# rishabhjain16/audio-visual-llm

Hardware: AMD Instinct MI355X
Metric: AV-clip train-step samples/sec (clip_whisper -> Llama-2-7B LoRA), whole job (higher is better)
Workload: dtype bf16

## Files before the change

### audio-visual-llm_amd/csrc/elementwise.hip

```cpp
#include "common.h"
#include "avllm_internal.h"

namespace {

template <typename T>
__global__ void rope_kernel(T* __restrict__ x, long ld, long rows, int T_, int heads, int hd, int pos0, float theta, int inverse) {
    const int half = hd >> 1;
    const long total = rows * heads * (half >> 2);
    for (long idx = blockIdx.x * (long)blockDim.x + threadIdx.x; idx < total; idx += (long)gridDim.x * blockDim.x) {
        const int qd = (int)(idx % (half >> 2));
        const int h = (int)((idx / (half >> 2)) % heads);
        const long row = idx / ((long)(half >> 2) * heads);
        const int pos = pos0 + (int)(row % T_);
        T* p = x + row * ld + (long)h * hd + qd * 4;
        float a[4], b[4], oa[4], ob[4];
        load_f<4>(p, a);
        load_f<4>(p + half, b);
#pragma unroll
        for (int j = 0; j < 4; ++j) {
            const int i = qd * 4 + j;
            const float inv = 1.0f / powf(theta, (float)(2 * i) / (float)hd);
            const float ang = (float)pos * inv;
            float c = cosf(ang), s = sinf(ang);
            if (inverse) s = -s;
// ... 206 lines not shown
        cols[(idx / w) * Kpad + K + idx % w] = from_f<T>(0.f);
}
template <typename T>
__global__ void cls_rows_kernel(const T* __restrict__ ce, const T* __restrict__ pos, T* __restrict__ x, int N, int tokens, int d) {
    const long total = (long)N * (d >> 2);
    for (long idx = blockIdx.x * (long)blockDim.x + threadIdx.x; idx < total; idx += (long)gridDim.x * blockDim.x) {
        const long n = idx / (d >> 2);
        const int c = (int)(idx % (d >> 2)) * 4;
        float a[4], b[4];
        load_f<4>(ce + c, a);
        load_f<4>(pos + c, b);
#pragma unroll
        for (int j = 0; j < 4; ++j) a[j] += b[j];
        store_f<4>(x + n * tokens * d + c, a);
    }
}

template <typename T>
__device__ __forceinline__ void virt_row(const T* a, int Ta, const T* v, int Tv, const T* pe, int P, int L, int b, int j, int c,
                                         int D, float fs, float (&o)[4]) {
    o[0] = o[1] = o[2] = o[3] = 0.f;
    if (j < P) { load_f<4>(pe + ((long)b * P + j) * D + c, o); return; }
    const int t = j - P;
    if (a && v) {
        float t4[4];
        if (t < Ta) { load_f<4>(a + ((long)b * Ta + t) * D + c, t4);
#pragma unroll
            for (int k = 0; k < 4; ++k) o[k] = fs * t4[k]; }
        if (t < Tv) { load_f<4>(v + ((long)b * Tv + t) * D + c, t4);
#pragma unroll
            for (int k = 0; k < 4; ++k) o[k] += (1.0f - fs) * t4[k]; }
    } else if (a) { if (t < Ta) load_f<4>(a + ((long)b * Ta + t) * D + c, o); }
    else { if (t < Tv) load_f<4>(v + ((long)b * Tv + t) * D + c, o); }
}

template <typename T>
__global__ void fuse_pool_kernel(const T* __restrict__ a, int Ta, const T* __restrict__ v, int Tv, const T* __restrict__ pe,
                                 int P, T* __restrict__ out, int L, int S_out, int D, float fs) {
    const int b = blockIdx.y, i = blockIdx.x;
    const int Lt = P + L;
    for (int c = threadIdx.x * 4; c < D; c += blockDim.x * 4) {
        float acc[4] = {0.f, 0.f, 0.f, 0.f}, r[4];
        if (Lt == S_out) {
            virt_row(a, Ta, v, Tv, pe, P, L, b, i, c, D, fs, acc);
        } else if (Lt > S_out) {
            const int s = (int)(((long)i * Lt) / S_out);
            const int e = (int)((((long)(i + 1)) * Lt + S_out - 1) / S_out);
            for (int j = s; j < e; ++j) {
                virt_row(a, Ta, v, Tv, pe, P, L, b, j, c, D, fs, r);
#pragma unroll
                for (int k = 0; k < 4; ++k) acc[k] += r[k];
            }
            const float cnt = (float)(e - s);
#pragma unroll
            for (int k = 0; k < 4; ++k) acc[k] = acc[k] / cnt;
        } else {
            const float scale = S_out > 1 ? (float)(Lt - 1) / (float)(S_out - 1) : 0.f;
            const float src = scale * i;
            const int lo = (int)src;
            const int hi = lo + 1 < Lt ? lo + 1 : Lt - 1;
            const float w1 = src - (float)lo, w0 = 1.0f - w1;
            float r2[4];
            virt_row(a, Ta, v, Tv, pe, P, L, b, lo, c, D, fs, r);
            virt_row(a, Ta, v, Tv, pe, P, L, b, hi, c, D, fs, r2);
#pragma unroll
            for (int k = 0; k < 4; ++k) acc[k] = w0 * r[k] + w1 * r2[k];
        }
        store_f<4>(out + ((long)b * S_out + i) * D + c, acc);
    }
}

template <typename T, int VEC>
__global__ void fuse_pool_bwd_kernel(const T* __restrict__ dx, T* __restrict__ da, int Ta, T* __restrict__ dv, int Tv, int P, int L,
                                     int S_out, int D, float fs) {
    const int b = blockIdx.y, t = blockIdx.x;
    const int Lt = P + L, j = P + t;
    const bool both = Ta > 0 && Tv > 0;
    const float scale = (Lt < S_out && S_out > 1) ? (float)(Lt - 1) / (float)(S_out - 1) : 0.f;
    int i0 = 0, i1 = -1;
    if (t < L) {
        if (Lt == S_out) { i0 = i1 = j; }
        else if (Lt > S_out) {
            i0 = (int)(((long)j * S_out) / Lt);
            i1 = (int)((((long)(j + 1)) * S_out - 1) / Lt);
        } else if (scale > 0.f) {
            i0 = (int)floorf((float)(j - 1) / scale) - 1;
            i1 = (int)ceilf((float)(j + 1) / scale) + 1;
        } else { i0 = 0; i1 = S_out - 1; }
        i0 = i0 < 0 ? 0 : i0;
        i1 = i1 > S_out - 1 ? S_out - 1 : i1;
    }
    for (int c = (int)threadIdx.x * VEC; c < D; c += (int)blockDim.x * VEC) {
        float g[VEC], r[VEC];
#pragma unroll
        for (int k = 0; k < VEC; ++k) g[k] = 0.f;
        for (int i = i0; i <= i1; ++i) {
            const T* src = dx + ((long)b * S_out + i) * D + c;
            if (Lt == S_out) {
                load_f<VEC>(src, g);
            } else if (Lt > S_out) {
                const int s = (int)(((long)i * Lt) / S_out);
                const int e = (int)((((long)(i + 1)) * Lt + S_out - 1) / S_out);
                if (j < s || j >= e) continue;
                const float cnt = (float)(e - s);
                load_f<VEC>(src, r);
#pragma unroll
                for (int k = 0; k < VEC; ++k) g[k] += r[k] / cnt;
            } else {
                const float sp = scale * i;
                const int lo = (int)sp;
                const int hi = lo + 1 < Lt ? lo + 1 : Lt - 1;
                if (lo != j && hi != j) continue;
                const float w1 = sp - (float)lo, w0 = 1.0f - w1;
                const float wgt = (lo == j ? w0 : 0.f) + (hi == j ? w1 : 0.f);
                load_f<VEC>(src, r);
#pragma unroll
                for (int k = 0; k < VEC; ++k) g[k] += wgt * r[k];
            }
        }
        if (da && t < Ta) {
#pragma unroll
            for (int k = 0; k < VEC; ++k) r[k] = both ? fs * g[k] : g[k];
            store_f<VEC>(da + ((long)b * Ta + t) * D + c, r);
        }
        if (dv && t < Tv) {
#pragma unroll
            for (int k = 0; k < VEC; ++k) r[k] = both ? (1.0f - fs) * g[k] : g[k];
            store_f<VEC>(dv + ((long)b * Tv + t) * D + c, r);
        }
    }
}

template <typename T>
__global__ void lora_pack_kernel(const float* __restrict__ A, const float* __restrict__ Bm, int r, int din, int dout,
                                 T* __restrict__ A_pad, T* __restrict__ AT_pad, long ld_at, T* __restrict__ B_pad, T* __restrict__ BT_pad) {
    const long nA = (long)AVLLM_LORA_PAD * din, nB = (long)AVLLM_LORA_PAD * dout;
    for (long idx = blockIdx.x * (long)blockDim.x + threadIdx.x; idx < nA + nB; idx += (long)gridDim.x * blockDim.x) {
        if (idx < nA) {
            const int j = (int)(idx / din), k = (int)(idx % din);
            const float val = j < r ? A[(long)j * din + k] : 0.f;
            A_pad[(long)j * din + k] = from_f<T>(val);
            AT_pad[(long)k * ld_at + j] = from_f<T>(val);
        } else {
            const long i2 = idx - nA;
            const int j = (int)(i2 / dout), n = (int)(i2 % dout);
            const float val = j < r ? Bm[(long)n * r + j] : 0.f;
            BT_pad[(long)j * dout + n] = from_f<T>(val);
            B_pad[(long)n * AVLLM_LORA_PAD + j] = from_f<T>(val);
        }
    }
}

template <typename T>
__global__ void lora_pack_batch_kernel(const avllm_lora_pack_item* __restrict__ items, int r, int din) {
    const avllm_lora_pack_item it = items[blockIdx.x];
    const int dout = (int)it.dout;
    const long nA = (long)r * din, nB = (long)r * dout;
    T* A_pad = (T*)it.A_pad; T* AT_pad = (T*)it.AT_pad; T* B_pad = (T*)it.B_pad; T* BT_pad = (T*)it.BT_pad;
    for (long idx = blockIdx.y * (long)blockDim.x + threadIdx.x; idx < nA + nB; idx += (long)gridDim.y * blockDim.x) {
        if (idx < nA) {
            const int j = (int)(idx / din), k = (int)(idx % din);
            const float val = it.A[(long)j * din + k];
            A_pad[(long)j * din + k] = from_f<T>(val);
            AT_pad[(long)k * it.ld_at + j] = from_f<T>(val);
        } else {
            const long i2 = idx - nA;
            const int j = (int)(i2 / dout), n = (int)(i2 % dout);
            const float val = it.B[(long)n * r + j];
            BT_pad[(long)j * dout + n] = from_f<T>(val);
            B_pad[(long)n * AVLLM_LORA_PAD + j] = from_f<T>(val);
        }
    }
}

template <typename T>
__global__ void kv_append_kernel(const T* __restrict__ k, const T* __restrict__ v, long ld, T* __restrict__ kc, T* __restrict__ vc,
                                 int B, int Tn, int pos0, int Tmax, int d) {
    const long total = (long)B * Tn * (d >> 2);
    for (long idx = blockIdx.x * (long)blockDim.x + threadIdx.x; idx < total; idx += (long)gridDim.x * blockDim.x) {
        const int c = (int)(idx % (d >> 2)) * 4;
        const long row = idx / (d >> 2);
        const int b = (int)(row / Tn), t = (int)(row % Tn);
        float x[4];
        load_f<4>(k + row * ld + c, x);
        store_f<4>(kc + ((long)b * Tmax + pos0 + t) * d + c, x);
        load_f<4>(v + row * ld + c, x);
        store_f<4>(vc + ((long)b * Tmax + pos0 + t) * d + c, x);
    }
}

inline int grid_for(long total, int block = 256) {
    long g = (total + block - 1) / block;
    return (int)(g < 1 ? 1 : (g > 8192 ? 8192 : g));
}

}

int av_rope(void* x, long ld, long rows, int T, int heads, int hd, int pos0, float theta, int inverse, int dtype, hipStream_t st) {
    AV_CHECK_ARG(x && rows > 0 && T > 0, "rope: null/empty");
    AV_CHECK_ARG(hd % 8 == 0 && ld % 4 == 0, "rope: head_dim %d must be a multiple of 8", hd);
    const long total = rows * heads * (hd / 8);
    if (dtype == AV_F32) hipLaunchKernelGGL((rope_kernel<float>), dim3(grid_for(total)), dim3(256), 0, st, (float*)x, ld, rows, T, heads, hd, pos0, theta, inverse);
    else hipLaunchKernelGGL((rope_kernel<bf16>), dim3(grid_for(total)), dim3(256), 0, st, (bf16*)x, ld, rows, T, heads, hd, pos0, theta, inverse);
    AV_LAUNCH_CHECK();
    return AV_OK;
}

int av_rope_table(float* tab, int T, int hd, int pos0, float theta, hipStream_t st, const int* pos_dev, AvRopeScale sc) {
    AV_CHECK_ARG(tab && T > 0 && hd % 8 == 0, "rope_table: bad args");
    hipLaunchKernelGGL(rope_table_kernel, dim3(av_cdiv((long)T * (hd / 2), 256)), dim3(256), 0, st, tab, T, hd, pos0, theta, pos_dev, sc);
    AV_LAUNCH_CHECK();
    return AV_OK;
}

int av_rope_tab(void* x, long ld, long rows, int T, int heads, int hd, const float* tab, int inverse, int dtype, hipStream_t st) {
    AV_CHECK_ARG(x && tab && rows > 0 && T > 0 && hd % 8 == 0 && ld % 4 == 0, "rope(tab): bad args");
    const long total = rows * heads * (hd / 8);
    if (dtype == AV_F32) hipLaunchKernelGGL((rope_tab_kernel<float>), dim3(grid_for(total)), dim3(256), 0, st, (float*)x, ld, rows, T, heads, hd, tab, inverse);
    else hipLaunchKernelGGL((rope_tab_kernel<bf16>), dim3(grid_for(total)), dim3(256), 0, st, (bf16*)x, ld, rows, T, heads, hd, tab, inverse);
    AV_LAUNCH_CHECK();
    return AV_OK;
}

int av_swiglu_fwd(const void* gu, void* h, long M, int F, int dtype, hipStream_t st) {
    AV_CHECK_ARG(gu && h && M > 0 && F % 4 == 0, "swiglu_fwd: bad args");
    if (dtype == AV_F32) hipLaunchKernelGGL((swiglu_fwd_kernel<float>), dim3(grid_for(M * (F / 4))), dim3(256), 0, st, (const float*)gu, (float*)h, M, F);
    else hipLaunchKernelGGL((swiglu_fwd_kernel<bf16>), dim3(grid_for(M * (F / 4))), dim3(256), 0, st, (const bf16*)gu, (bf16*)h, M, F);
    AV_LAUNCH_CHECK();
    return AV_OK;
}

int av_swiglu_bwd(const void* dh, const void* gu, void* dgu, long M, int F, int dtype, hipStream_t st) {
    AV_CHECK_ARG(dh && gu && dgu && M > 0 && F % 4 == 0, "swiglu_bwd: bad args");
    if (dtype == AV_F32) hipLaunchKernelGGL((swiglu_bwd_kernel<float, false>), dim3(grid_for(M * (F / 4))), dim3(256), 0, st, (const float*)dh, (const float*)gu, (float*)dgu, (float*)nullptr, M, F);
    else hipLaunchKernelGGL((swiglu_bwd_kernel<bf16, false>), dim3(grid_for(M * (F / 4))), dim3(256), 0, st, (const bf16*)dh, (const bf16*)gu, (bf16*)dgu, (bf16*)nullptr, M, F);
    AV_LAUNCH_CHECK();
    return AV_OK;
}

int av_swiglu_bwd_h(const void* dh, const void* gu, void* dgu, void* h, long M, int F, int dtype, hipStream_t st) {
    AV_CHECK_ARG(dh && gu && dgu && h && M > 0 && F > 0 && F % 4 == 0, "swiglu_bwd_h: bad args");
    AV_CHECK_ARG(dtype == AV_F32 || dtype == AV_BF16, "swiglu_bwd_h: dtype %d", dtype);
    if (dtype == AV_F32) hipLaunchKernelGGL((swiglu_bwd_kernel<float, true>), dim3(grid_for(M * (F / 4))), dim3(256), 0, st, (const float*)dh, (const float*)gu, (float*)dgu, (float*)h, M, F);
    else hipLaunchKernelGGL((swiglu_bwd_kernel<bf16, true>), dim3(grid_for(M * (F / 4))), dim3(256), 0, st, (const bf16*)dh, (const bf16*)gu, (bf16*)dgu, (bf16*)h, M, F);
    AV_LAUNCH_CHECK();
    return AV_OK;
}

int av_act_residual(const void* x, const void* r, void* y, long n, int act, int dtype, hipStream_t st) {
    AV_CHECK_ARG(x && y && n > 0 && n % 4 == 0, "act_residual: bad args (n=%ld must be a multiple of 4)", n);
    if (dtype == AV_F32) hipLaunchKernelGGL((act_residual_kernel<float>), dim3(grid_for(n / 4)), dim3(256), 0, st, (const float*)x, (const float*)r, (float*)y, n / 4, act);
    else hipLaunchKernelGGL((act_residual_kernel<bf16>), dim3(grid_for(n / 4)), dim3(256), 0, st, (const bf16*)x, (const bf16*)r, (bf16*)y, n / 4, act);
    AV_LAUNCH_CHECK();
    return AV_OK;
}

int av_dropout(const void* x, void* y, long rows, int d, uint32_t seed, float p, int dtype, hipStream_t st, const uint32_t* seed_dev) {
    AV_CHECK_ARG(x && y && rows > 0 && d % 4 == 0 && p >= 0.f && p < 1.f, "dropout: bad args");
    const long total = rows * (d / 4);
    if (dtype == AV_F32) hipLaunchKernelGGL((dropout_kernel<float>), dim3(grid_for(total)), dim3(256), 0, st, (const float*)x, (float*)y, rows, d, seed, p, seed_dev);
    else hipLaunchKernelGGL((dropout_kernel<bf16>), dim3(grid_for(total)), dim3(256), 0, st, (const bf16*)x, (bf16*)y, rows, d, seed, p, seed_dev);
    AV_LAUNCH_CHECK();
    return AV_OK;
}

int av_embedding(const void* table, const int64_t* ids, void* out, long n, int d, int dtype, hipStream_t st) {
    AV_CHECK_ARG(table && ids && out && n > 0 && d % 4 == 0, "embedding: bad args");
    if (dtype == AV_F32) hipLaunchKernelGGL((embedding_kernel<float>), dim3(grid_for(n * (d / 4))), dim3(256), 0, st, (const float*)table, ids, (float*)out, n, d);
    else hipLaunchKernelGGL((embedding_kernel<bf16>), dim3(grid_for(n * (d / 4))), dim3(256), 0, st, (const bf16*)table, ids, (bf16*)out, n, d);
    AV_LAUNCH_CHECK();
    return AV_OK;
}

int av_cast(const void* src, int sdt, void* dst, int ddt, long n, hipStream_t st) {
    AV_CHECK_ARG(src && dst && n > 0, "cast: bad args");
    const dim3 g(grid_for(n / 4 + 1)), b(256);
    if (sdt == AV_F32 && ddt == AV_BF16) hipLaunchKernelGGL((cast_kernel<float, bf16>), g, b, 0, st, (const float*)src, (bf16*)dst, n);
    else if (sdt == AV_BF16 && ddt == AV_F32) hipLaunchKernelGGL((cast_kernel<bf16, float>), g, b, 0, st, (const bf16*)src, (float*)dst, n);
    else if (sdt == AV_F32 && ddt == AV_F32) hipLaunchKernelGGL((cast_kernel<float, float>), g, b, 0, st, (const float*)src, (float*)dst, n);
    else if (sdt == AV_BF16 && ddt == AV_BF16) hipLaunchKernelGGL((cast_kernel<bf16, bf16>), g, b, 0, st, (const bf16*)src, (bf16*)dst, n);
    else return av_set_error(AV_ERR_ARG, "cast: dtype %d->%d", sdt, ddt);
    AV_LAUNCH_CHECK();
    return AV_OK;
}

int av_whisper_im2col1(const float* mel, void* cols, int B, int n_mels, int T, int Kpad, int dtype, hipStream_t st) {
    AV_CHECK_ARG(mel && cols && B > 0 && T > 0, "im2col1: bad args");
    AV_CHECK_ARG(Kpad % 4 == 0 && Kpad >= n_mels * 3, "im2col1: Kpad=%d too small", Kpad);
    const size_t sh = (size_t)n_mels * 68 * sizeof(float);
    if (dtype == AV_F32) hipLaunchKernelGGL((im2col1_kernel<float>), dim3(av_cdiv(T, 64), B), dim3(256), sh, st, mel, (float*)cols, n_mels, T, Kpad);
    else hipLaunchKernelGGL((im2col1_kernel<bf16>), dim3(av_cdiv(T, 64), B), dim3(256), sh, st, mel, (bf16*)cols, n_mels, T, Kpad);
    AV_LAUNCH_CHECK();
    return AV_OK;
}

int av_whisper_im2col2(const void* h, void* cols, int B, int T, int d, int dtype, hipStream_t st) {
    AV_CHECK_ARG(h && cols && B > 0 && T % 2 == 0 && d % 8 == 0, "im2col2: bad args");
    const long total = (long)B * (T / 2) * 3 * (d / 8);
    if (dtype == AV_F32) hipLaunchKernelGGL((im2col2_kernel<float>), dim3(grid_for(total)), dim3(256), 0, st, (const float*)h, (float*)cols, B, T, d);
    else hipLaunchKernelGGL((im2col2_kernel<bf16>), dim3(grid_for(total)), dim3(256), 0, st, (const bf16*)h, (bf16*)cols, B, T, d);
    AV_LAUNCH_CHECK();
    return AV_OK;
}

int av_clip_patchify(const void* frames, void* cols, int N, int S, int p, int Kpad, int dtype, hipStream_t st, int in_dtype) {
    AV_CHECK_ARG(frames && cols && N > 0, "patchify: bad args");
    AV_CHECK_ARG(p > 0 && S % p == 0, "patchify: image %d is not a whole number of %d-pixel patches", S, p);
    const int K = 3 * p * p;
    AV_CHECK_ARG(Kpad >= K && Kpad % 4 == 0, "patchify: Kpad=%d < %d", Kpad, K);
    const int V = p % 4 == 0 ? 4 : p % 2 == 0 ? 2 : 1;
    const long total = (long)N * 3 * S * (S / V);
    const long rows = (long)N * (S / p) * (S / p);
#define AV_PATCHIFY(T, VV) do { if (in_dtype == AV_BF16) hipLaunchKernelGGL((patchify_kernel<T, VV, bf16>), dim3(grid_for(total)), dim3(256), 0, st, (const bf16*)frames, (T*)cols, N, S, p, Kpad); \
                                else hipLaunchKernelGGL((patchify_kernel<T, VV, float>), dim3(grid_for(total)), dim3(256), 0, st, (const float*)frames, (T*)cols, N, S, p, Kpad); } while (0)
    if (dtype == AV_F32) {
        if (V == 4) AV_PATCHIFY(float, 4); else if (V == 2) AV_PATCHIFY(float, 2); else AV_PATCHIFY(float, 1);
        if (Kpad > K) hipLaunchKernelGGL((patchify_pad_kernel<float>), dim3(grid_for(rows * (Kpad - K))), dim3(256), 0, st, (float*)cols, rows, K, Kpad);
    } else {
        if (V == 4) AV_PATCHIFY(bf16, 4); else if (V == 2) AV_PATCHIFY(bf16, 2); else AV_PATCHIFY(bf16, 1);
        if (Kpad > K) hipLaunchKernelGGL((patchify_pad_kernel<bf16>), dim3(grid_for(rows * (Kpad - K))), dim3(256), 0, st, (bf16*)cols, rows, K, Kpad);
    }
#undef AV_PATCHIFY
    AV_LAUNCH_CHECK();
// ... 67 lines not shown
```

### audio-visual-llm_amd/csrc/lora_batch.hip

```cpp
#include "common.h"
#include "avllm_internal.h"

namespace {

constexpr int RK_WAVES = 8;

struct Rank3Args {
    const bf16* A[3]; long lda[3]; int K[3];
    const bf16* B[3]; long ldb[3];
    bf16* C[3]; long ldc[3];
    uint32_t seed[3];
    int nj, M;
    float alpha, p;
    const uint32_t* seed_dev;
};

__device__ __forceinline__ bf16x8 rk_drop(bf16x8 x, uint32_t seed, unsigned long long idx0, uint32_t thr, float sc) {
    float v[8];
#pragma unroll
    for (int j = 0; j < 8; ++j) v[j] = (float)x[j];
    av_mask8(v, seed, idx0, thr, sc);
    bf16x8 r;
#pragma unroll
    for (int j = 0; j < 8; ++j) r[j] = (bf16)v[j];
    return r;
}

template <bool SHARED, bool DROP, int NJ>
__global__ __launch_bounds__(RK_WAVES * 64) void lora_rank3_kernel(Rank3Args a) {
    __shared__ float part[NJ][RK_WAVES][16][17];
    const int lane = threadIdx.x & 63, w = threadIdx.x >> 6;
    const int fr = lane & 15, fq = lane >> 4;
    const int m0 = blockIdx.x * 16;
    const int j0 = SHARED ? 0 : blockIdx.y;
    int ar = m0 + fr; ar = ar < a.M ? ar : a.M - 1;
    const int K = a.K[j0], kw = K / RK_WAVES;
    const bf16* ap = a.A[j0] + (long)ar * a.lda[j0] + (long)w * kw + fq * 8;
    const bf16* bp[NJ];
    uint32_t seed[NJ];
    f32x4 acc[NJ];
#pragma unroll
    for (int j = 0; j < NJ; ++j) {
        bp[j] = a.B[j0 + j] + (long)fr * a.ldb[j0 + j] + (long)w * kw + fq * 8;
        seed[j] = DROP ? av_seed(a.seed_dev, a.seed[j0 + j]) : 0u;
        acc[j] = (f32x4){0.f, 0.f, 0.f, 0.f};
    }
    const uint32_t thr = av_drop_thr(a.p);
    const float dsc = av_drop_scale(a.p);
    const unsigned long long idx_base = (unsigned long long)ar * K + (unsigned long long)w * kw + fq * 8;
    constexpr int UNR = 4;
    int k = 0;
    for (; k + 32 * UNR <= kw; k += 32 * UNR) {
        bf16x8 xa[UNR], wb[UNR][NJ];
#pragma unroll
        for (int u = 0; u < UNR; ++u) {
            xa[u] = *(const bf16x8*)(ap + k + 32 * u);
#pragma unroll
            for (int j = 0; j < NJ; ++j) wb[u][j] = *(const bf16x8*)(bp[j] + k + 32 * u);
        }
#pragma unroll
        for (int u = 0; u < UNR; ++u)
#pragma unroll
            for (int j = 0; j < NJ; ++j) {
                const bf16x8 x = DROP ? rk_drop(xa[u], seed[j], idx_base + k + 32 * u, thr, dsc) : xa[u];
                acc[j] = __builtin_amdgcn_mfma_f32_16x16x32_bf16(wb[u][j], x, acc[j], 0, 0, 0);
            }
    }
    for (; k < kw; k += 32) {
        const bf16x8 xa = *(const bf16x8*)(ap + k);
#pragma unroll
        for (int j = 0; j < NJ; ++j) {
            const bf16x8 wb = *(const bf16x8*)(bp[j] + k);
            const bf16x8 x = DROP ? rk_drop(xa, seed[j], idx_base + k, thr, dsc) : xa;
            acc[j] = __builtin_amdgcn_mfma_f32_16x16x32_bf16(wb, x, acc[j], 0, 0, 0);
        }
    }
#pragma unroll
    for (int j = 0; j < NJ; ++j)
#pragma unroll
        for (int i = 0; i < 4; ++i) part[j][w][fr][fq * 4 + i] = acc[j][i];
    __syncthreads();
    for (int e = threadIdx.x; e < NJ * 16 * 64; e += RK_WAVES * 64) {
        const int j = e / (16 * 64), r = (e >> 6) & 15, c = e & 63;
        if (m0 + r >= a.M) continue;
        float s = 0.f;
        if (c < 16) {
#pragma unroll
            for (int x = 0; x < RK_WAVES; ++x) s += part[j][x][r][c];
            s *= a.alpha;
        }
        a.C[j0 + j][(long)(m0 + r) * a.ldc[j0 + j] + c] = (bf16)s;
    }
}

typedef __attribute__((address_space(3))) short4v* lds_s4_ptr;
typedef __attribute__((ext_vector_type(8))) short short8v;

__device__ __forceinline__ bf16x8 tn_frag16(const char* img, int stride, int row0, int col0, int lane) {
    const int g = lane >> 4, i16 = lane & 15;
    const char* a0 = img + (row0 + 8 * g + (i16 >> 2)) * stride + (col0 + 4 * (i16 & 3)) * 2;
    const short4v lo = __builtin_amdgcn_ds_read_tr16_b64_v4i16((lds_s4_ptr)(a0));
    const short4v hi = __builtin_amdgcn_ds_read_tr16_b64_v4i16((lds_s4_ptr)(a0 + 4 * stride));
    const short8v both = {lo[0], lo[1], lo[2], lo[3], hi[0], hi[1], hi[2], hi[3]};
    return __builtin_bit_cast(bf16x8, both);
}

constexpr int TM_N = 128, TM_M = 64, TM_BIG = TM_N * 2 + 64, TM_SM = 48;

struct TnMultiArgs {
    const bf16* Big; long ldb; int NB;
    const bf16* Small[3]; long lds[3];
    float* out[3]; long ldo[3];
    int col0[3], ncol[3];
    uint32_t seed[3];
    int nj, R, M, mchunk;
    float alpha, p;
    const uint32_t* seed_dev;
};

template <bool SHARED, int NJ>
__global__ __launch_bounds__(256) void gemm_tn_multi_kernel(TnMultiArgs a) {
    extern __shared__ __attribute__((aligned(16))) char tm_smem[];
    char* big_s = tm_smem;
    char* small_s = tm_smem + NJ * TM_M * TM_BIG;
    const int tid = threadIdx.x, lane = tid & 63, w = tid >> 6;
    const int n0 = blockIdx.x * TM_N;
    int j0 = 0;
    if (!SHARED) j0 = (a.nj > 1 && n0 >= a.col0[1]) + (a.nj > 2 && n0 >= a.col0[2]);
    const int m_begin = blockIdx.y * a.mchunk, m_end = min(a.M, m_begin + a.mchunk);
    const bool drop = SHARED && a.p > 0.f;
    uint32_t seed[NJ];
#pragma unroll
    for (int j = 0; j < NJ; ++j) seed[j] = drop ? av_seed(a.seed_dev, a.seed[j]) : 0u;
    f32x4 acc[NJ][2];
#pragma unroll
    for (int j = 0; j < NJ; ++j) { acc[j][0] = (f32x4){0.f, 0.f, 0.f, 0.f}; acc[j][1] = (f32x4){0.f, 0.f, 0.f, 0.f}; }
    constexpr int BPT = TM_M * (TM_N / 8) / 256;
    u32x4 nb[BPT], ns[NJ];
    auto fetch = [&](int mb) {
#pragma unroll
        for (int i = 0; i < BPT; ++i) {
            const int c = tid + i * 256, row = c >> 4, ch = c & 15;
            nb[i] = (u32x4){0u, 0u, 0u, 0u};
            if (mb + row < m_end) nb[i] = *(const u32x4*)(a.Big + (long)(mb + row) * a.ldb + n0 + ch * 8);
        }
        if (tid < TM_M * 2) {
            const int row = tid >> 1, ch = tid & 1;
#pragma unroll
            for (int j = 0; j < NJ; ++j) {
                ns[j] = (u32x4){0u, 0u, 0u, 0u};
                if (mb + row < m_end) ns[j] = *(const u32x4*)(a.Small[j0 + j] + (long)(mb + row) * a.lds[j0 + j] + ch * 8);
            }
        }
    };
    if (m_begin < m_end) fetch(m_begin);
    const uint32_t thr = av_drop_thr(a.p);
    const float dsc = av_drop_scale(a.p);
    for (int mb = m_begin; mb < m_end; mb += TM_M) {
        __syncthreads();
#pragma unroll
        for (int i = 0; i < BPT; ++i) {
            const int c = tid + i * 256, row = c >> 4, ch = c & 15;
            if (drop) {
                const bf16x8 xb = __builtin_bit_cast(bf16x8, nb[i]);
#pragma unroll
                for (int j = 0; j < NJ; ++j) {
                    float f[8];
#pragma unroll
                    for (int q = 0; q < 8; ++q) f[q] = (float)xb[q];
                    av_mask8(f, seed[j], (unsigned long long)(mb + row) * a.NB + n0 + ch * 8, thr, dsc);
                    bf16x8 yb;
#pragma unroll
                    for (int q = 0; q < 8; ++q) yb[q] = (bf16)f[q];
                    *(u32x4*)(big_s + j * TM_M * TM_BIG + row * TM_BIG + ch * 16) = __builtin_bit_cast(u32x4, yb);
                }
            } else {
                *(u32x4*)(big_s + row * TM_BIG + ch * 16) = nb[i];
            }
        }
        if (tid < TM_M * 2) {
#pragma unroll
            for (int j = 0; j < NJ; ++j) *(u32x4*)(small_s + j * TM_M * TM_SM + (tid >> 1) * TM_SM + (tid & 1) * 16) = ns[j];
        }
        __syncthreads();
        if (mb + TM_M < m_end) fetch(mb + TM_M);
#pragma unroll
        for (int ks = 0; ks < TM_M / 32; ++ks) {
#pragma unroll
            for (int j = 0; j < NJ; ++j) {
                const bf16x8 sa = tn_frag16(small_s + j * TM_M * TM_SM, TM_SM, 32 * ks, 0, lane);
                const char* img = big_s + (drop ? j * TM_M * TM_BIG : 0);
#pragma unroll
                for (int t = 0; t < 2; ++t) {
                    const bf16x8 bb = tn_frag16(img, TM_BIG, 32 * ks, w * 32 + t * 16, lane);
                    acc[j][t] = __builtin_amdgcn_mfma_f32_16x16x32_bf16(sa, bb, acc[j][t], 0, 0, 0);
                }
            }
        }
    }
    const int fr = lane & 15, fq = lane >> 4;
#pragma unroll
    for (int j = 0; j < NJ; ++j)
#pragma unroll
        for (int t = 0; t < 2; ++t) {
            const int n = n0 + w * 32 + t * 16 + fr;
#pragma unroll
            for (int i = 0; i < 4; ++i) {
                const int r = fq * 4 + i;
                if (r < a.R) {
                    float* p = SHARED ? a.out[j] + (long)r * a.ldo[j] + n : a.out[j0] + (long)(n - a.col0[j0]) * a.ldo[j0] + r;
                    atomicAdd(p, a.alpha * acc[j][t][i]);
                }
            }
        }
}

int tn_chunks(int M, int want, int& mchunk) {
    int zs = av_cdiv(M, want);
    zs = zs > 32 ? 32 : zs;
    mchunk = av_cdiv(M, zs);
    mchunk = (mchunk + TM_M - 1) / TM_M * TM_M;
    return av_cdiv(M, mchunk);
}

}

bool av_lora_batch_supported(int dtype, int R, int nj) { return dtype == AV_BF16 && R >= 1 && R <= 16 && nj >= 1 && nj <= 3; }

int av_lora_rank3(const void* const* A, const long* lda, const int* K, const void* const* B, const long* ldb, void* const* C, const long* ldc,
                  const uint32_t* seeds, int nj, int M, int R, float alpha, float p, const uint32_t* seed_dev, int shared, int dtype, hipStream_t st) {
    AV_CHECK_ARG(A && lda && K && B && ldb && C && ldc && M > 0, "lora_rank3: null/empty");
    AV_CHECK_ARG(av_lora_batch_supported(dtype, R, nj), "lora_rank3: bf16, rank <= 16 (r=%d), 1..3 adapters (nj=%d)", R, nj);
    AV_CHECK_ARG(p >= 0.f && p < 1.f && (p == 0.f || shared), "lora_rank3: dropout (p=%f) only on the shared-input form", p);
    Rank3Args a = {};
    for (int j = 0; j < nj; ++j) {
        const int ja = shared ? 0 : j;
        AV_CHECK_ARG(A[ja] && B[j] && C[j], "lora_rank3: null operand %d", j);
        AV_CHECK_ARG(K[ja] > 0 && K[ja] % (32 * RK_WAVES) == 0 && lda[ja] % 8 == 0 && ldb[j] % 8 == 0 && ldc[j] >= 64,
                     "lora_rank3: K %% 256 == 0 (K=%d), 16-byte rows, 64-wide outputs", K[ja]);
        AV_CHECK_ARG(p == 0.f || lda[ja] == K[ja], "lora_rank3: the fused mask needs the full contiguous [M,K] activation as A");
        a.A[j] = (const bf16*)A[ja]; a.lda[j] = lda[ja]; a.K[j] = K[ja]; a.B[j] = (const bf16*)B[j]; a.ldb[j] = ldb[j];
        a.C[j] = (bf16*)C[j]; a.ldc[j] = ldc[j]; a.seed[j] = seeds ? seeds[j] : 0u;
    }
    a.nj = nj; a.M = M; a.alpha = alpha; a.p = p; a.seed_dev = seed_dev;
    const int gx = av_cdiv(M, 16);
    const dim3 blk(RK_WAVES * 64);
#define RK_LAUNCH(SH, DR, NJV, GY) hipLaunchKernelGGL((lora_rank3_kernel<SH, DR, NJV>), dim3(gx, GY), blk, 0, st, a)
    if (shared) {
        if (p > 0.f) { if (nj == 3) RK_LAUNCH(true, true, 3, 1); else if (nj == 2) RK_LAUNCH(true, true, 2, 1); else RK_LAUNCH(true, true, 1, 1); }
        else { if (nj == 3) RK_LAUNCH(true, false, 3, 1); else if (nj == 2) RK_LAUNCH(true, false, 2, 1); else RK_LAUNCH(true, false, 1, 1); }
    } else RK_LAUNCH(false, false, 1, nj);
#undef RK_LAUNCH
    AV_LAUNCH_CHECK();
    return AV_OK;
}

int av_gemm_tn_multi(const void* Big, long ldb, int NB, const void* const* Small, const long* lds, float* const* out, const long* ldo,
                     const int* col0, const int* ncol, const uint32_t* seeds, int nj, int R, int M, float alpha, float p,
                     const uint32_t* seed_dev, int shared, int dtype, hipStream_t st) {
    AV_CHECK_ARG(Big && Small && lds && out && ldo && M > 0 && NB > 0 && NB % TM_N == 0 && ldb % 8 == 0, "gemm_tn_multi: bad args (NB=%d)", NB);
    AV_CHECK_ARG(av_lora_batch_supported(dtype, R, nj), "gemm_tn_multi: bf16, rank <= 16 (r=%d), 1..3 adapters (nj=%d)", R, nj);
    AV_CHECK_ARG(p >= 0.f && p < 1.f && (p == 0.f || shared), "gemm_tn_multi: dropout (p=%f) only on the shared form", p);
    TnMultiArgs a = {};
    a.Big = (const bf16*)Big; a.ldb = ldb; a.NB = NB;
    int next = 0;
    for (int j = 0; j < nj; ++j) {
        AV_CHECK_ARG(Small[j] && out[j] && lds[j] % 8 == 0 && lds[j] >= 16, "gemm_tn_multi: operand %d", j);
        a.Small[j] = (const bf16*)Small[j]; a.lds[j] = lds[j]; a.out[j] = out[j]; a.ldo[j] = ldo[j]; a.seed[j] = seeds ? seeds[j] : 0u;
        if (!shared) {
            AV_CHECK_ARG(col0 && ncol && col0[j] == next && ncol[j] > 0 && ncol[j] % TM_N == 0, "gemm_tn_multi: column ranges must tile [0, NB) in 128-column units");
            a.col0[j] = col0[j]; a.ncol[j] = ncol[j]; next += ncol[j];
        }
    }
    AV_CHECK_ARG(shared || next == NB, "gemm_tn_multi: column ranges cover %d of %d columns", next, NB);
    a.nj = nj; a.R = R; a.M = M; a.alpha = alpha; a.p = p; a.seed_dev = seed_dev;
    const int zs = tn_chunks(M, shared ? 256 : 512, a.mchunk);
    const dim3 grid(NB / TM_N, zs);
    const int njk = shared ? nj : 1;
    const size_t lds_bytes = (size_t)njk * TM_M * (TM_BIG + TM_SM);
    static bool attr[64][3] = {};
    int dev = 0;
    AV_HIP(hipGetDevice(&dev));
#define TM_LAUNCH(SH, NJV) do { \
        if (!attr[dev & 63][NJV - 1] && SH) { AV_HIP(hipFuncSetAttribute((const void*)gemm_tn_multi_kernel<SH, NJV>, hipFuncAttributeMaxDynamicSharedMemorySize, (int)lds_bytes)); attr[dev & 63][NJV - 1] = true; } \
        hipLaunchKernelGGL((gemm_tn_multi_kernel<SH, NJV>), grid, dim3(256), lds_bytes, st, a); } while (0)
    if (shared) { if (nj == 3) TM_LAUNCH(true, 3); else if (nj == 2) TM_LAUNCH(true, 2); else TM_LAUNCH(true, 1); }
    else TM_LAUNCH(false, 1);
#undef TM_LAUNCH
    AV_LAUNCH_CHECK();
    return AV_OK;
}

extern "C" int avllm_lora_rank3(const void* const* A, const int64_t* lda, const int32_t* K, const void* const* B, const int64_t* ldb, void* const* C,
                                const int64_t* ldc, const uint32_t* seeds, int32_t nj, int32_t M, int32_t R, float alpha, float p,
                                const uint32_t* seed_dev, int32_t shared, int32_t dtype, void* stream) {
    AV_CHECK_ARG(nj >= 1 && nj <= 3 && lda && K && ldb && ldc, "lora_rank3: nj=%d", nj);
    long la[3], lb[3], lc[3]; int kk[3];
    for (int j = 0; j < nj; ++j) { la[j] = (long)lda[j]; lb[j] = (long)ldb[j]; lc[j] = (long)ldc[j]; kk[j] = K[j]; }
    return av_lora_rank3(A, la, kk, B, lb, C, lc, seeds, nj, M, R, alpha, p, seed_dev, shared, dtype, (hipStream_t)stream);
}

extern "C" int avllm_gemm_tn_multi(const void* Big, int64_t ldb, int32_t NB, const void* const* Small, const int64_t* lds, float* const* out,
                                   const int64_t* ldo, const int32_t* col0, const int32_t* ncol, const uint32_t* seeds, int32_t nj, int32_t R,
                                   int32_t M, float alpha, float p, const uint32_t* seed_dev, int32_t shared, int32_t dtype, void* stream) {
    AV_CHECK_ARG(nj >= 1 && nj <= 3 && lds && ldo, "gemm_tn_multi: nj=%d", nj);
    long ls[3], lo[3]; int c0[3] = {0, 0, 0}, nc[3] = {0, 0, 0};
    for (int j = 0; j < nj; ++j) { ls[j] = (long)lds[j]; lo[j] = (long)ldo[j]; if (col0) c0[j] = col0[j]; if (ncol) nc[j] = ncol[j]; }
    return av_gemm_tn_multi(Big, ldb, NB, Small, ls, out, lo, col0 ? c0 : nullptr, ncol ? nc : nullptr, seeds, nj, R, M, alpha, p, seed_dev, shared,
                            dtype, (hipStream_t)stream);
}
```

### audio-visual-llm_amd/csrc/lora_dx.hip

```cpp
#include "common.h"
#include "avllm_internal.h"

namespace {

constexpr int DX_ROWS = 32, DX_COLS = 128;

struct LoraDxArgs {
    const bf16* T[3]; const bf16* AT[3];
    long ldt[3], ldat[3];
    uint32_t seed[3];
    const bf16* R; bf16* out;
    long ldr, ldo;
    int M, N, nj;
    float p;
    const uint32_t* seed_dev;
};

__device__ __forceinline__ void mask4_add(f32x4& acc, const f32x4 v, uint32_t seed, unsigned long long idx0, uint32_t thr, float sc) {
    const uint32_t h0 = av_pair_hash(seed, idx0 >> 1), h1 = av_pair_hash(seed, (idx0 >> 1) + 1);
    acc[0] += (h0 & 0xffffu) >= thr ? v[0] * sc : 0.f;
    acc[1] += (h0 >> 16) >= thr ? v[1] * sc : 0.f;
    acc[2] += (h1 & 0xffffu) >= thr ? v[2] * sc : 0.f;
    acc[3] += (h1 >> 16) >= thr ? v[3] * sc : 0.f;
}

template <int NJ>
__global__ __launch_bounds__(256) void lora_dx_masked_kernel(LoraDxArgs a) {
    __shared__ __attribute__((aligned(16))) float lds[4 * DX_ROWS * DX_COLS];
    const int lane = threadIdx.x & 63, wave = threadIdx.x >> 6;
    const int fr = lane & 15, fq = lane >> 4;
    const int m0 = (blockIdx.y * 4 + wave) * DX_ROWS, n0 = blockIdx.x * DX_COLS;
    if (m0 >= a.M) return;
    float* cw = lds + wave * DX_ROWS * DX_COLS;
    const uint32_t thr = av_drop_thr(a.p);
    const float sc = av_drop_scale(a.p);
    uint32_t seed[NJ];
#pragma unroll
    for (int j = 0; j < NJ; ++j) seed[j] = av_seed(a.seed_dev, a.seed[j]);
    bf16x8 xa[2][NJ];
#pragma unroll
    for (int rb = 0; rb < 2; ++rb) {
        int m = m0 + rb * 16 + fr;
        m = m < a.M ? m : a.M - 1;
#pragma unroll
        for (int j = 0; j < NJ; ++j) xa[rb][j] = *(const bf16x8*)(a.T[j] + (long)m * a.ldt[j] + fq * 8);
    }
#pragma unroll 2
    for (int ct = 0; ct < DX_COLS / 16; ++ct) {
        bf16x8 wb[NJ];
#pragma unroll
        for (int j = 0; j < NJ; ++j) wb[j] = *(const bf16x8*)(a.AT[j] + (long)(n0 + ct * 16 + fr) * a.ldat[j] + fq * 8);
#pragma unroll
        for (int rb = 0; rb < 2; ++rb) {
            f32x4 acc = {0.f, 0.f, 0.f, 0.f};
            const int row = rb * 16 + fr;
            const unsigned long long idx0 = (unsigned long long)(m0 + row) * a.N + n0 + ct * 16 + 4 * fq;
#pragma unroll
            for (int j = 0; j < NJ; ++j) {
                const f32x4 z = {0.f, 0.f, 0.f, 0.f};
                const f32x4 pj = __builtin_amdgcn_mfma_f32_16x16x32_bf16(wb[j], xa[rb][j], z, 0, 0, 0);
                mask4_add(acc, pj, seed[j], idx0, thr, sc);
            }
            *(f32x4*)(cw + row * DX_COLS + (((ct * 4 + fq) ^ (row & 7)) << 2)) = acc;
        }
    }
    asm volatile("s_waitcnt lgkmcnt(0)" ::: "memory");
#pragma unroll
    for (int i = 0; i < DX_ROWS * (DX_COLS / 8) / 64; ++i) {
        const int c = lane + 64 * i, row = c >> 4, ch = c & 15;
        const int m = m0 + row;
        const f32x4 lo = *(const f32x4*)(cw + row * DX_COLS + (((2 * ch) ^ (row & 7)) << 2));
        const f32x4 hi = *(const f32x4*)(cw + row * DX_COLS + (((2 * ch + 1) ^ (row & 7)) << 2));
        if (m < a.M) {
            float v[8] = {lo[0], lo[1], lo[2], lo[3], hi[0], hi[1], hi[2], hi[3]};
            if (a.R) {
                const bf16x8 r = *(const bf16x8*)(a.R + (long)m * a.ldr + n0 + ch * 8);
#pragma unroll
                for (int q = 0; q < 8; ++q) v[q] += (float)r[q];
            }
            store_f<8>(a.out + (long)m * a.ldo + n0 + ch * 8, v);
        }
    }
}

}

bool av_lora_dx_masked_supported(int dtype, int N, int r, const long* ldt, const long* ldat, int nj, long ldr, long ldo) {
    if (dtype != AV_BF16 || N % DX_COLS != 0 || r > 32 || nj < 1 || nj > 3 || ldr % 8 != 0 || ldo % 8 != 0) return false;
    for (int j = 0; j < nj; ++j)
        if (ldt[j] % 8 != 0 || ldat[j] % 8 != 0 || ldt[j] < 32 || ldat[j] < 32) return false;
    return true;
}

int av_lora_dx_masked(const void* const* T, const long* ldt, const void* const* AT, const long* ldat, const uint32_t* seeds, int nj, int r,
                      const void* R, long ldr, void* out, long ldo, int M, int N, float p, const uint32_t* seed_dev, int dtype, hipStream_t st) {
    AV_CHECK_ARG(T && AT && ldt && ldat && seeds && out && M > 0 && N > 0, "lora_dx_masked: null/empty");
    AV_CHECK_ARG(av_lora_dx_masked_supported(dtype, N, r, ldt, ldat, nj, R ? ldr : 8, ldo),
                 "lora_dx_masked: bf16 only, N %% 128 == 0 (N=%d), rank <= 32 (r=%d), 1..3 adapters (nj=%d), 16-byte rows", N, r, nj);
    AV_CHECK_ARG(p >= 0.f && p < 1.f, "lora_dx_masked: p=%f", p);
    LoraDxArgs a = {};
    for (int j = 0; j < nj; ++j) {
        AV_CHECK_ARG(T[j] && AT[j], "lora_dx_masked: null adapter %d", j);
        a.T[j] = (const bf16*)T[j]; a.AT[j] = (const bf16*)AT[j]; a.ldt[j] = ldt[j]; a.ldat[j] = ldat[j]; a.seed[j] = seeds[j];
    }
    a.R = (const bf16*)R; a.out = (bf16*)out; a.ldr = ldr; a.ldo = ldo; a.M = M; a.N = N; a.nj = nj; a.p = p; a.seed_dev = seed_dev;
    const dim3 grid(N / DX_COLS, av_cdiv(M, 4 * DX_ROWS));
    if (nj == 1) hipLaunchKernelGGL(lora_dx_masked_kernel<1>, grid, dim3(256), 0, st, a);
    else if (nj == 2) hipLaunchKernelGGL(lora_dx_masked_kernel<2>, grid, dim3(256), 0, st, a);
    else hipLaunchKernelGGL(lora_dx_masked_kernel<3>, grid, dim3(256), 0, st, a);
    AV_LAUNCH_CHECK();
    return AV_OK;
}

extern "C" int avllm_lora_dx_masked(const void* const* T, const int64_t* ldt, const void* const* AT, const int64_t* ldat, const uint32_t* seeds,
                                    int32_t nj, int32_t r, const void* R, int64_t ldr, void* out, int64_t ldo, int32_t M, int32_t N, float p,
                                    const uint32_t* seed_dev, int32_t dtype, void* stream) {
    AV_CHECK_ARG(nj >= 1 && nj <= 3 && ldt && ldat, "lora_dx_masked: nj=%d", nj);
    long lt[3], la[3];
    for (int j = 0; j < nj; ++j) { lt[j] = (long)ldt[j]; la[j] = (long)ldat[j]; }
    return av_lora_dx_masked(T, lt, AT, la, seeds, nj, r, R, ldr, out, ldo, M, N, p, seed_dev, dtype, (hipStream_t)stream);
}
```

Measured before the change: 91.73.

## Tile LoRA pack, deepen TN prefetch pipeline, narrow dx tiles with early loads

The LoRA pack kernel now works on 8x8 tiles with vectorized loads and stores for both the plain and transposed copies, replacing scalar strided writes. The non-shared TN multi-GEMM path keeps four slabs of global loads in flight in registers so memory latency overlaps the MFMA work. The LoRA dx kernel halves its column tile to 64, adds an occupancy hint, and hoists the residual and weight-fragment loads ahead of compute. In exchange, all three kernels use more registers per thread, which may lower occupancy.

```diff
diff --git a/audio-visual-llm_amd/csrc/elementwise.hip b/audio-visual-llm_amd/csrc/elementwise.hip
--- a/audio-visual-llm_amd/csrc/elementwise.hip
+++ b/audio-visual-llm_amd/csrc/elementwise.hip
@@ -382,23 +382,48 @@
 }
 
 template <typename T>
+__device__ __forceinline__ void pack_tile8(const float* __restrict__ S, long lds, int rows, int cols, int r0, int c0, T* __restrict__ D, long ldd,
+                                           T* __restrict__ DT, long ldt, bool vec) {
+    if (vec && r0 + 8 <= rows && c0 + 8 <= cols) {
+        float v[8][8];
+#pragma unroll
+        for (int i = 0; i < 8; ++i) load_f<8>(S + (long)(r0 + i) * lds + c0, v[i]);
+#pragma unroll
+        for (int i = 0; i < 8; ++i) store_f<8>(D + (long)(r0 + i) * ldd + c0, v[i]);
+#pragma unroll
+        for (int c = 0; c < 8; ++c) {
+            const float t[8] = {v[0][c], v[1][c], v[2][c], v[3][c], v[4][c], v[5][c], v[6][c], v[7][c]};
+            store_f<8>(DT + (long)(c0 + c) * ldt + r0, t);
+        }
+        return;
+    }
+    for (int i = 0; i < 8 && r0 + i < rows; ++i)
+        for (int c = 0; c < 8 && c0 + c < cols; ++c) {
+            const T val = from_f<T>(S[(long)(r0 + i) * lds + c0 + c]);
+            D[(long)(r0 + i) * ldd + c0 + c] = val;
+            DT[(long)(c0 + c) * ldt + r0 + i] = val;
+        }
+}
+
+__device__ __forceinline__ bool pack_vec_ok(const void* p, long ld_elems, int elem_bytes) {
+    return ((uintptr_t)p & 15) == 0 && (ld_elems * elem_bytes) % 16 == 0;
+}
+
+template <typename T>
 __global__ void lora_pack_batch_kernel(const avllm_lora_pack_item* __restrict__ items, int r, int din) {
     const avllm_lora_pack_item it = items[blockIdx.x];
     const int dout = (int)it.dout;
-    const long nA = (long)r * din, nB = (long)r * dout;
     T* A_pad = (T*)it.A_pad; T* AT_pad = (T*)it.AT_pad; T* B_pad = (T*)it.B_pad; T* BT_pad = (T*)it.BT_pad;
-    for (long idx = blockIdx.y * (long)blockDim.x + threadIdx.x; idx < nA + nB; idx += (long)gridDim.y * blockDim.x) {
-        if (idx < nA) {
-            const int j = (int)(idx / din), k = (int)(idx % din);
-            const float val = it.A[(long)j * din + k];
-            A_pad[(long)j * din + k] = from_f<T>(val);
-            AT_pad[(long)k * it.ld_at + j] = from_f<T>(val);
+    const int rt = (r + 7) / 8, kt = (din + 7) / 8, nt = (dout + 7) / 8;
+    const bool vecA = pack_vec_ok(it.A, din, 4) && pack_vec_ok(A_pad, din, sizeof(T)) && pack_vec_ok(AT_pad, it.ld_at, sizeof(T));
+    const bool vecB = pack_vec_ok(it.B, r, 4) && pack_vec_ok(B_pad, AVLLM_LORA_PAD, sizeof(T)) && pack_vec_ok(BT_pad, dout, sizeof(T));
+    const long nA = (long)rt * kt, nB = (long)nt * rt;
+    for (long t = blockIdx.y * (long)blockDim.x + threadIdx.x; t < nA + nB; t += (long)gridDim.y * blockDim.x) {
+        if (t < nA) {
+            pack_tile8<T>(it.A, din, r, din, (int)(t / kt) * 8, (int)(t % kt) * 8, A_pad, din, AT_pad, it.ld_at, vecA);
         } else {
-            const long i2 = idx - nA;
-            const int j = (int)(i2 / dout), n = (int)(i2 % dout);
-            const float val = it.B[(long)n * r + j];
-            BT_pad[(long)j * dout + n] = from_f<T>(val);
-            B_pad[(long)n * AVLLM_LORA_PAD + j] = from_f<T>(val);
+            const long t2 = t - nA;
+            pack_tile8<T>(it.B, r, dout, r, (int)(t2 / rt) * 8, (int)(t2 % rt) * 8, B_pad, AVLLM_LORA_PAD, BT_pad, dout, vecB);
         }
     }
 }
diff --git a/audio-visual-llm_amd/csrc/lora_batch.hip b/audio-visual-llm_amd/csrc/lora_batch.hip
--- a/audio-visual-llm_amd/csrc/lora_batch.hip
+++ b/audio-visual-llm_amd/csrc/lora_batch.hip
@@ -106,6 +106,24 @@
 }
 
 constexpr int TM_N = 128, TM_M = 64, TM_BIG = TM_N * 2 + 64, TM_SM = 48;
+constexpr int TM_DEPTH = 4;
+
+template <int NJ>
+__device__ __forceinline__ void tn_slab_mma(const char* small_s, const char* big_s, bool drop, int lane, int w, f32x4 (&acc)[NJ][2]) {
+#pragma unroll
+    for (int ks = 0; ks < TM_M / 32; ++ks) {
+#pragma unroll
+        for (int j = 0; j < NJ; ++j) {
+            const bf16x8 sa = tn_frag16(small_s + j * TM_M * TM_SM, TM_SM, 32 * ks, 0, lane);
+            const char* img = big_s + (drop ? j * TM_M * TM_BIG : 0);
+#pragma unroll
+            for (int t = 0; t < 2; ++t) {
+                const bf16x8 bb = tn_frag16(img, TM_BIG, 32 * ks, w * 32 + t * 16, lane);
+                acc[j][t] = __builtin_amdgcn_mfma_f32_16x16x32_bf16(sa, bb, acc[j][t], 0, 0, 0);
+            }
+        }
+    }
+}
 
 struct TnMultiArgs {
     const bf16* Big; long ldb; int NB;
@@ -136,65 +154,101 @@
 #pragma unroll
     for (int j = 0; j < NJ; ++j) { acc[j][0] = (f32x4){0.f, 0.f, 0.f, 0.f}; acc[j][1] = (f32x4){0.f, 0.f, 0.f, 0.f}; }
     constexpr int BPT = TM_M * (TM_N / 8) / 256;
-    u32x4 nb[BPT], ns[NJ];
-    auto fetch = [&](int mb) {
-#pragma unroll
-        for (int i = 0; i < BPT; ++i) {
-            const int c = tid + i * 256, row = c >> 4, ch = c & 15;
-            nb[i] = (u32x4){0u, 0u, 0u, 0u};
-            if (mb + row < m_end) nb[i] = *(const u32x4*)(a.Big + (long)(mb + row) * a.ldb + n0 + ch * 8);
-        }
-        if (tid < TM_M * 2) {
-            const int row = tid >> 1, ch = tid & 1;
-#pragma unroll
-            for (int j = 0; j < NJ; ++j) {
-                ns[j] = (u32x4){0u, 0u, 0u, 0u};
-                if (mb + row < m_end) ns[j] = *(const u32x4*)(a.Small[j0 + j] + (long)(mb + row) * a.lds[j0 + j] + ch * 8);
-            }
-        }
-    };
-    if (m_begin < m_end) fetch(m_begin);
-    const uint32_t thr = av_drop_thr(a.p);
-    const float dsc = av_drop_scale(a.p);
-    for (int mb = m_begin; mb < m_end; mb += TM_M) {
-        __syncthreads();
-#pragma unroll
-        for (int i = 0; i < BPT; ++i) {
-            const int c = tid + i * 256, row = c >> 4, ch = c & 15;
-            if (drop) {
-                const bf16x8 xb = __builtin_bit_cast(bf16x8, nb[i]);
+    if constexpr (SHARED) {
+        u32x4 nb[BPT], ns[NJ];
+        auto fetch = [&](int mb) {
+#pragma unroll
+            for (int i = 0; i < BPT; ++i) {
+                const int c = tid + i * 256, row = c >> 4, ch = c & 15;
+                nb[i] = (u32x4){0u, 0u, 0u, 0u};
+                if (mb + row < m_end) nb[i] = *(const u32x4*)(a.Big + (long)(mb + row) * a.ldb + n0 + ch * 8);
+            }
+            if (tid < TM_M * 2) {
+                const int row = tid >> 1, ch = tid & 1;
 #pragma unroll
                 for (int j = 0; j < NJ; ++j) {
-                    float f[8];
-#pragma unroll
-                    for (int q = 0; q < 8; ++q) f[q] = (float)xb[q];
-                    av_mask8(f, seed[j], (unsigned long long)(mb + row) * a.NB + n0 + ch * 8, thr, dsc);
-                    bf16x8 yb;
-#pragma unroll
-                    for (int q = 0; q < 8; ++q) yb[q] = (bf16)f[q];
-                    *(u32x4*)(big_s + j * TM_M * TM_BIG + row * TM_BIG + ch * 16) = __builtin_bit_cast(u32x4, yb);
-                }
-            } else {
-                *(u32x4*)(big_s + row * TM_BIG + ch * 16) = nb[i];
-            }
-        }
-        if (tid < TM_M * 2) {
-#pragma unroll
-            for (int j = 0; j < NJ; ++j) *(u32x4*)(small_s + j * TM_M * TM_SM + (tid >> 1) * TM_SM + (tid & 1) * 16) = ns[j];
-        }
-        __syncthreads();
-        if (mb + TM_M < m_end) fetch(mb + TM_M);
-#pragma unroll
-        for (int ks = 0; ks < TM_M / 32; ++ks) {
-#pragma unroll
-            for (int j = 0; j < NJ; ++j) {
-                const bf16x8 sa = tn_frag16(small_s + j * TM_M * TM_SM, TM_SM, 32 * ks, 0, lane);
-                const char* img = big_s + (drop ? j * TM_M * TM_BIG : 0);
-#pragma unroll
-                for (int t = 0; t < 2; ++t) {
-                    const bf16x8 bb = tn_frag16(img, TM_BIG, 32 * ks, w * 32 + t * 16, lane);
-                    acc[j][t] = __builtin_amdgcn_mfma_f32_16x16x32_bf16(sa, bb, acc[j][t], 0, 0, 0);
-                }
+                    ns[j] = (u32x4){0u, 0u, 0u, 0u};
+                    if (mb + row < m_end) ns[j] = *(const u32x4*)(a.Small[j0 + j] + (long)(mb + row) * a.lds[j0 + j] + ch * 8);
+                }
+            }
+        };
+        if (m_begin < m_end) fetch(m_begin);
+        const uint32_t thr = av_drop_thr(a.p);
+        const float dsc = av_drop_scale(a.p);
+        for (int mb = m_begin; mb < m_end; mb += TM_M) {
+            __syncthreads();
+#pragma unroll
+            for (int i = 0; i < BPT; ++i) {
+                const int c = tid + i * 256, row = c >> 4, ch = c & 15;
+                if (drop) {
+                    const bf16x8 xb = __builtin_bit_cast(bf16x8, nb[i]);
+#pragma unroll
+                    for (int j = 0; j < NJ; ++j) {
+                        float f[8];
+#pragma unroll
+                        for (int q = 0; q < 8; ++q) f[q] = (float)xb[q];
+                        av_mask8(f, seed[j], (unsigned long long)(mb + row) * a.NB + n0 + ch * 8, thr, dsc);
+                        bf16x8 yb;
+#pragma unroll
+                        for (int q = 0; q < 8; ++q) yb[q] = (bf16)f[q];
+                        *(u32x4*)(big_s + j * TM_M * TM_BIG + row * TM_BIG + ch * 16) = __builtin_bit_cast(u32x4, yb);
+                    }
+                } else {
+                    *(u32x4*)(big_s + row * TM_BIG + ch * 16) = nb[i];
+                }
+            }
+            if (tid < TM_M * 2) {
+#pragma unroll
+                for (int j = 0; j < NJ; ++j) *(u32x4*)(small_s + j * TM_M * TM_SM + (tid >> 1) * TM_SM + (tid & 1) * 16) = ns[j];
+            }
+            __syncthreads();
+            if (mb + TM_M < m_end) fetch(mb + TM_M);
+#pragma unroll
+            for (int ks = 0; ks < TM_M / 32; ++ks) {
+#pragma unroll
+                for (int j = 0; j < NJ; ++j) {
+                    const bf16x8 sa = tn_frag16(small_s + j * TM_M * TM_SM, TM_SM, 32 * ks, 0, lane);
+                    const char* img = big_s + (drop ? j * TM_M * TM_BIG : 0);
+#pragma unroll
+                    for (int t = 0; t < 2; ++t) {
+                        const bf16x8 bb = tn_frag16(img, TM_BIG, 32 * ks, w * 32 + t * 16, lane);
+                        acc[j][t] = __builtin_amdgcn_mfma_f32_16x16x32_bf16(sa, bb, acc[j][t], 0, 0, 0);
+                    }
+                }
+            }
+        }
+    } else {
+        u32x4 nb[TM_DEPTH][BPT], ns[TM_DEPTH];
+        auto fetch = [&](const int s, const int mb) __attribute__((always_inline)) {
+#pragma unroll
+            for (int i = 0; i < BPT; ++i) {
+                const int c = tid + i * 256, row = c >> 4, ch = c & 15;
+                nb[s][i] = (u32x4){0u, 0u, 0u, 0u};
+                if (mb + row < m_end) nb[s][i] = *(const u32x4*)(a.Big + (long)(mb + row) * a.ldb + n0 + ch * 8);
+            }
+            if (tid < TM_M * 2) {
+                ns[s] = (u32x4){0u, 0u, 0u, 0u};
+                if (mb + (tid >> 1) < m_end) ns[s] = *(const u32x4*)(a.Small[j0] + (long)(mb + (tid >> 1)) * a.lds[j0] + (tid & 1) * 8);
+            }
+        };
+#pragma unroll
+        for (int s = 0; s < TM_DEPTH; ++s)
+            if (m_begin + s * TM_M < m_end) fetch(s, m_begin + s * TM_M);
+        for (int mb0 = m_begin; mb0 < m_end; mb0 += TM_DEPTH * TM_M) {
+#pragma unroll
+            for (int s = 0; s < TM_DEPTH; ++s) {
+                const int mb = mb0 + s * TM_M;
+                if (mb >= m_end) break;
+                __syncthreads();
+#pragma unroll
+                for (int i = 0; i < BPT; ++i) {
+                    const int c = tid + i * 256, row = c >> 4, ch = c & 15;
+                    *(u32x4*)(big_s + row * TM_BIG + ch * 16) = nb[s][i];
+                }
+                if (tid < TM_M * 2) *(u32x4*)(small_s + (tid >> 1) * TM_SM + (tid & 1) * 16) = ns[s];
+                __syncthreads();
+                if (mb + TM_DEPTH * TM_M < m_end) fetch(s, mb + TM_DEPTH * TM_M);
+                tn_slab_mma<NJ>(small_s, big_s, false, lane, w, acc);
             }
         }
     }
diff --git a/audio-visual-llm_amd/csrc/lora_dx.hip b/audio-visual-llm_amd/csrc/lora_dx.hip
--- a/audio-visual-llm_amd/csrc/lora_dx.hip
+++ b/audio-visual-llm_amd/csrc/lora_dx.hip
@@ -3,7 +3,8 @@
 
 namespace {
 
-constexpr int DX_ROWS = 32, DX_COLS = 128;
+constexpr int DX_ROWS = 32, DX_COLS = 64;
+constexpr int DX_N_UNIT = 128, DX_CPR = DX_COLS / 8;
 
 struct LoraDxArgs {
     const bf16* T[3]; const bf16* AT[3];
@@ -25,7 +26,7 @@
 }
 
 template <int NJ>
-__global__ __launch_bounds__(256) void lora_dx_masked_kernel(LoraDxArgs a) {
+__global__ __launch_bounds__(256, 4) void lora_dx_masked_kernel(LoraDxArgs a) {
     __shared__ __attribute__((aligned(16))) float lds[4 * DX_ROWS * DX_COLS];
     const int lane = threadIdx.x & 63, wave = threadIdx.x >> 6;
     const int fr = lane & 15, fq = lane >> 4;
@@ -37,6 +38,15 @@
     uint32_t seed[NJ];
 #pragma unroll
     for (int j = 0; j < NJ; ++j) seed[j] = av_seed(a.seed_dev, a.seed[j]);
+    constexpr int NCH = DX_ROWS * (DX_COLS / 8) / 64;
+    bf16x8 res[NCH];
+    if (a.R) {
+#pragma unroll
+        for (int i = 0; i < NCH; ++i) {
+            const int c = lane + 64 * i, m = m0 + c / DX_CPR;
+            if (m < a.M) res[i] = *(const bf16x8*)(a.R + (long)m * a.ldr + n0 + (c % DX_CPR) * 8);
+        }
+    }
     bf16x8 xa[2][NJ];
 #pragma unroll
     for (int rb = 0; rb < 2; ++rb) {
@@ -45,11 +55,13 @@
 #pragma unroll
         for (int j = 0; j < NJ; ++j) xa[rb][j] = *(const bf16x8*)(a.T[j] + (long)m * a.ldt[j] + fq * 8);
     }
-#pragma unroll 2
+    bf16x8 wb[DX_COLS / 16][NJ];
+#pragma unroll
+    for (int ct = 0; ct < DX_COLS / 16; ++ct)
+#pragma unroll
+        for (int j = 0; j < NJ; ++j) wb[ct][j] = *(const bf16x8*)(a.AT[j] + (long)(n0 + ct * 16 + fr) * a.ldat[j] + fq * 8);
+#pragma unroll
     for (int ct = 0; ct < DX_COLS / 16; ++ct) {
-        bf16x8 wb[NJ];
-#pragma unroll
-        for (int j = 0; j < NJ; ++j) wb[j] = *(const bf16x8*)(a.AT[j] + (long)(n0 + ct * 16 + fr) * a.ldat[j] + fq * 8);
 #pragma unroll
         for (int rb = 0; rb < 2; ++rb) {
             f32x4 acc = {0.f, 0.f, 0.f, 0.f};
@@ -58,7 +70,7 @@
 #pragma unroll
             for (int j = 0; j < NJ; ++j) {
                 const f32x4 z = {0.f, 0.f, 0.f, 0.f};
-                const f32x4 pj = __builtin_amdgcn_mfma_f32_16x16x32_bf16(wb[j], xa[rb][j], z, 0, 0, 0);
+                const f32x4 pj = __builtin_amdgcn_mfma_f32_16x16x32_bf16(wb[ct][j], xa[rb][j], z, 0, 0, 0);
                 mask4_add(acc, pj, seed[j], idx0, thr, sc);
             }
             *(f32x4*)(cw + row * DX_COLS + (((ct * 4 + fq) ^ (row & 7)) << 2)) = acc;
@@ -66,17 +78,16 @@
     }
     asm volatile("s_waitcnt lgkmcnt(0)" ::: "memory");
 #pragma unroll
-    for (int i = 0; i < DX_ROWS * (DX_COLS / 8) / 64; ++i) {
-        const int c = lane + 64 * i, row = c >> 4, ch = c & 15;
+    for (int i = 0; i < NCH; ++i) {
+        const int c = lane + 64 * i, row = c / DX_CPR, ch = c % DX_CPR;
         const int m = m0 + row;
         const f32x4 lo = *(const f32x4*)(cw + row * DX_COLS + (((2 * ch) ^ (row & 7)) << 2));
         const f32x4 hi = *(const f32x4*)(cw + row * DX_COLS + (((2 * ch + 1) ^ (row & 7)) << 2));
         if (m < a.M) {
             float v[8] = {lo[0], lo[1], lo[2], lo[3], hi[0], hi[1], hi[2], hi[3]};
             if (a.R) {
-                const bf16x8 r = *(const bf16x8*)(a.R + (long)m * a.ldr + n0 + ch * 8);
 #pragma unroll
-                for (int q = 0; q < 8; ++q) v[q] += (float)r[q];
+                for (int q = 0; q < 8; ++q) v[q] += (float)res[i][q];
             }
             store_f<8>(a.out + (long)m * a.ldo + n0 + ch * 8, v);
         }
@@ -86,7 +97,7 @@
 }
 
 bool av_lora_dx_masked_supported(int dtype, int N, int r, const long* ldt, const long* ldat, int nj, long ldr, long ldo) {
-    if (dtype != AV_BF16 || N % DX_COLS != 0 || r > 32 || nj < 1 || nj > 3 || ldr % 8 != 0 || ldo % 8 != 0) return false;
+    if (dtype != AV_BF16 || N % DX_N_UNIT != 0 || r > 32 || nj < 1 || nj > 3 || ldr % 8 != 0 || ldo % 8 != 0) return false;
     for (int j = 0; j < nj; ++j)
         if (ldt[j] % 8 != 0 || ldat[j] % 8 != 0 || ldt[j] < 32 || ldat[j] < 32) return false;
     return true;
```

Result: no change. 92.17, median of 6 (+0.5%).
